# mkln/spamtree

Measured on AMD Instinct MI355X. Metric: Gibbs iterations/sec + achieved HBM GB/s, n=1e6 grid, 1/2/4/8 MI355X, higher is better.
Workload: dtype f64

## Files before the change

spamtree_amd/csrc/misc_kernels.hpp:

```cpp
#pragma once
#include "st_device.hpp"

struct LoglikArgs {
  const Blk *blks;
  const int *anc_idx;
  const int *list;
  int nlist;
  const double *panels;
  const double *w;
  double *loglik_c;
  double *resid;
  int maxP, maxM;
};

struct LoglikGrpArgs {
  const Blk *blks;
  const int *anc_idx;
  const Grp *grps;
  const int *list;
  int nlist;
  const double *panels;
  const double *w;
  double *loglik_c;
  int maxP;
// ... 176 lines not shown
  for (int i = lo + threadIdx.x; i < hi; i += NT) { xa += a[i]; xb += b[i]; }
  sa[threadIdx.x] = xa; sb[threadIdx.x] = xb;
  __syncthreads();
  for (int s2 = NT / 2; s2 > 0; s2 >>= 1) {
    if ((int)threadIdx.x < s2) { sa[threadIdx.x] += sa[threadIdx.x + s2]; sb[threadIdx.x] += sb[threadIdx.x + s2]; }
    __syncthreads();
  }
  if (threadIdx.x == 0) { partial[2 * blockIdx.x] = sa[0]; partial[2 * blockIdx.x + 1] = sb[0]; }
}
__global__ void k_sum2_final(const double *partial, double *out) {
  if (threadIdx.x < 2) {
    double s2 = 0.0;
    for (int g = 0; g < SUM2_WG; ++g) s2 += partial[2 * g + threadIdx.x];
    out[threadIdx.x] = s2;
  }
}

__global__ void k_xb(const double *X, const int *mv, const double *B, long long n, int p, double *xb) {
  const long long i = (long long)blockIdx.x * blockDim.x + threadIdx.x;
  if (i >= n) return;
  const double *bj = B + (size_t)p * mv[i];
  double acc = 0.0;
  for (int j = 0; j < p; ++j) acc += X[(size_t)j * n + i] * bj[j];
  xb[i] = acc;
}

template <int Q, bool XTX>
__global__ __launch_bounds__(NT) void k_stats(const double *X, const double *y, const double *w, const double *xb, const int *mv,
                                               const unsigned char *obs, const long long *partner, const double *wt, long long n,
                                               int p, double *partial) {
// ... 153 lines not shown
  const long long i = (long long)blockIdx.x * blockDim.x + threadIdx.x;
  if (i < n) buf[i] = mask[i] ? w[i] : 0.0;
  if (i < world) buf[n + i] = (i == rank && err[0] != INT_MAX) ? (double)err[0] : 0.0;
}

__global__ void k_merge_err(int *err, const int *err2) {
  if (threadIdx.x == 0 && blockIdx.x == 0 && err2[0] < err[0]) err[0] = err2[0];
}

#else
__global__ void k_normals(double *z, const long long *dev2model, long long n, unsigned iter, unsigned stream, unsigned long long seed);
__global__ void k_loglik(LoglikArgs A);
__global__ void k_loglik_grp(LoglikGrpArgs A);
__global__ void k_sum2_partial(const double *a, const double *b, int n, double *partial);
__global__ void k_sum2_final(const double *partial, double *out);
__global__ void k_xb(const double *X, const int *mv, const double *B, long long n, int p, double *xb);
template <int Q, bool XTX> __global__ void k_stats(const double *X, const double *y, const double *w, const double *xb, const int *mv, const unsigned char *obs, const long long *partner, const double *wt, long long n, int p, double *partial);
__global__ void k_stats_final(const double *partial, int nwg, int nq, double *out);
__global__ void k_yhat(const double *xb, const double *w, const double *noise, const int *mv, long long n, const double *tsq_inv_q, double *yhat);
__global__ void k_cross_cov(const double *c1, const int *mv1, long long n1, const double *c2, const int *mv2, long long n2, CovPar cp, double *out);
__global__ void k_qtile(QtArgs A);
__global__ void k_axpy_sum(double *acc, const double *x, long long n);
__global__ void k_pack_comps(const double *logdet, const double *loglik, const unsigned char *mask, int nb, const int *err, int rank, int world, double *buf);
__global__ void k_gather_pack(const double *w, const int *idx, int cnt, const int *err, double *out);
__global__ void k_gather_unpack(const double *recv, const int *idx, int cnt, long long total, double *w, double *errs);
__global__ void k_pack_w(const double *w, const unsigned char *mask, long long n, const int *err, int rank, int world, double *buf);
__global__ void k_merge_err(int *err, const int *err2);
#endif

static void launch_sum2(hipStream_t st, const double *a, const double *b, int n, double *partial, double *out) {
  hipLaunchKernelGGL(k_sum2_partial, dim3(SUM2_WG), dim3(NT), 0, st, a, b, n, partial);
  hipLaunchKernelGGL(k_sum2_final, dim3(1), dim3(64), 0, st, partial, out);
}
```

spamtree_amd/csrc/spamtree_hip.hip:

```cpp

#include "st_handle.hpp"
#include "misc_kernels.hpp"
#include "draw_store.hpp"
#include "rows_score.hpp"
#include <new>

static thread_local std::string g_create_error;
void points_free(st_handle_s *h);

enum RouteCode : int {
  R_NONE = ST_ROUTE_NONE,
  R_MARGINAL_INVCHOL_WAVE, R_MARGINAL_INVCHOL,
  R_FACTOR_LDS, R_FACTOR_SCRATCH, R_PREDICT_LDS, R_PREDICT_SCRATCH,
  R_QUAD32_REF_WCH, R_QUAD32_REF, R_QUAD32_LEAF, R_QUAD38_REF_WCH, R_QUAD38_REF, R_QUAD38_LEAF,
  R_QUAD44_REF_WCH, R_QUAD44_REF, R_QUAD44_LEAF, R_QUAD50_REF_WCH, R_QUAD50_REF, R_QUAD50_LEAF,
  R_FACTOR_MFMA, R_LCHAIN96, R_LCHAIN136, R_REF_FINISH, R_LCHAIN_SCALARS, R_FACTOR_WIDE, R_BIGMFMA3, R_BIGMFMA4, R_BIGMFMA5,
  R_GRAM, R_GRAM_DIRECT, R_GRAM_BIG,
  R_SAMPLE_MFMA, R_LEAF_SEG4, R_LEAF_SEG6, R_SAMPLE_LEAF, R_SAMPLE_WAVE, R_SAMPLE_LEAN_LAT, R_SAMPLE_LEAN,
  R_SAMPLE_BIG_REF, R_SAMPLE_LEAF_WIDE, R_SAMPLE_BIG_LEAF, R_SAMPLE_SMALL,
  R_COUNT
};
static const char *const k_route_names[R_COUNT] = {
  "",
  "k_marginal_invchol_wave", "k_marginal_invchol",
// ... 42 lines not shown
  return tab[size][kind];
}
static int launch_quad(int nkx, bool isref, bool wave_chol, int nquad, size_t lds, hipStream_t st, const QuadArgs &F, const CovPar &cp) {
  const int size = nkx == 32 ? 0 : nkx == 38 ? 1 : nkx == 44 ? 2 : 3, kind = isref ? (wave_chol ? 0 : 1) : 2;
  hipLaunchKernelGGL(quad_kernel(size, kind), dim3(nquad), dim3(128 * 4), lds, st, F, cp);
  return R_QUAD32_REF_WCH + QUAD_KINDS * size + kind;
}

static void invalidate_stats(st_handle_s *h) {
  if (h->stats_on_stream2) {
    (void)hipSetDevice(h->device);
    (void)hipStreamWaitEvent(h->stream, h->ev_stats, 0);
    h->stats_on_stream2 = false;
  }
  h->stats_valid = false; h->host_stats_valid = false;
}


extern "C" const char *st_last_error(st_handle h) { return h ? h->err.c_str() : g_create_error.c_str(); }
extern "C" void st_set_create_error(const char *msg) { g_create_error = msg ? msg : ""; }

extern "C" int st_destroy(st_handle h) {
  if (!h) return ST_OK;
  (void)hipSetDevice(h->device);
  if (h->ev_top) (void)hipEventDestroy(h->ev_top);
  if (h->ev_main) (void)hipEventDestroy(h->ev_main);
  if (h->ev_stats) (void)hipEventDestroy(h->ev_stats);
  if (h->stream2) (void)hipStreamDestroy(h->stream2);
  prof_harvest(h);
  for (auto e : h->ev_free) (void)hipEventDestroy(e);
  if (h->comm) (void)ncclCommDestroy(h->comm);
  if (h->pin) (void)hipHostFree(h->pin);
  if (h->pin_up) (void)hipHostFree(h->pin_up);
  for (int i = 0; i < 2; ++i) if (h->ev_up[i]) (void)hipEventDestroy(h->ev_up[i]);
  if (h->ev_factor) (void)hipEventDestroy(h->ev_factor);
  points_free(h);
  if (h->stream && !h->ext_stream) (void)hipStreamDestroy(h->stream);
  delete h;
  return ST_OK;
}

extern "C" int st_shard_plan_opt(const st_problem *pb, const st_options *opt_in, int32_t world, int64_t *owner, int32_t *cut_level) {
// ... 53 lines not shown
  for (long long r = 0; r < n; ++r)
    if (std::isfinite(pb->y[r])) rank_av[r] = t++;
  for (long long i = 0; i < n; ++i) {
    const long long r = h->dev2model[i];
    partner[i] = (h->quirks && rank_av[r] >= 0) ? h->model2dev[rank_av[r]] : i;
  }
  h->xtx.assign((size_t)pb->p * pb->p * pb->q, 0.0);
  for (long long r = 0; pb->p <= 8 && r < n; ++r) {
    if (!std::isfinite(pb->y[r])) continue;
    const int v = (int)(pb->mv_id[r] - 1);
    for (int a = 0; a < pb->p; ++a)
      for (int b2 = 0; b2 < pb->p; ++b2)
        h->xtx[(size_t)v * pb->p * pb->p + (size_t)b2 * pb->p + a] += pb->X[(size_t)a * n + r] * pb->X[(size_t)b2 * n + r];
  }
  CCHK(hipStreamCreate(&h->stream));
  CCHK(hipHostMalloc((void **)&h->pin, sizeof(PinnedArea), hipHostMallocDefault));
  new (h->pin) PinnedArea();
  h->pin_up_len = QMAX + std::max(1, h->p * h->q);
  CCHK(hipHostMalloc((void **)&h->pin_up, (size_t)2 * h->pin_up_len * sizeof(double), hipHostMallocDefault));
  for (int i = 0; i < 2; ++i) CCHK(hipEventCreateWithFlags(&h->ev_up[i], hipEventDisableTiming));
  CCHK(hipEventCreateWithFlags(&h->ev_factor, hipEventDisableTiming));
  CCHK(h->d_cx.upload(cx)); CCHK(h->d_cy.upload(cy)); CCHK(h->d_y.upload(y)); CCHK(h->d_X.upload(X));
  CCHK(h->d_mv.upload(mv)); CCHK(h->d_obs.upload(obs)); CCHK(h->d_partner.upload(partner));
  CCHK(h->d_dev2model.upload(h->dev2model));
  return ST_OK;
}

static int create_layout_buffers(st_handle_s *h) {
  {
    std::vector<Blk> db = h->blks;
    if (h->limited) for (Blk &B : db) B.acc_len = 0;
    CCHK(h->d_blks.upload(db));
// ... 33 lines not shown
  CCHK(h->d_resid.alloc(n));
  CCHK(hipMemset(h->d_resid.p, 0, n * sizeof(double)));
  CCHK(h->d_B.alloc((size_t)h->p * h->q));
  CCHK(h->d_tsq.alloc(QMAX));
  for (int s = 0; s < 2; ++s) {
    CCHK(h->d_panels[s].alloc(h->panel_total + 128));
    CCHK(hipMemset(h->d_panels[s].p, 0, (h->panel_total + 128) * sizeof(double)));
    CCHK(h->d_logdet[s].alloc(nb)); CCHK(h->d_loglik[s].alloc(nb));
    CCHK(hipMemset(h->d_logdet[s].p, 0, nb * sizeof(double)));
    CCHK(hipMemset(h->d_loglik[s].p, 0, nb * sizeof(double)));
  }
  CCHK(h->d_acc.alloc(std::max<size_t>(h->acc_total, 1)));
  CCHK(hipMemset(h->d_acc.p, 0, std::max<size_t>(h->acc_total, 1) * sizeof(double)));
  CCHK(h->d_scalars.alloc(8 + 2 * SUM2_WG));
  CCHK(h->d_err.alloc(2));
  CCHK(h->d_partial.alloc((size_t)STATS_WG * (h->p * h->q + h->q)));
  CCHK(h->d_stats.alloc((size_t)h->p * h->q + h->q));
  if (h->p <= 8) return ST_OK;
  const int p = h->p, pq = p * h->q;
  CCHK(h->d_xtx.alloc((size_t)p * pq));
  for (int b2 = 0; b2 < p; ++b2) {
    launch_stats(h, h->stream, h->d_X.p + (size_t)b2 * n);
    hipLaunchKernelGGL(k_stats_final, dim3(pq), dim3(NT), 0, h->stream, h->d_partial.p, STATS_WG, pq + h->q, h->d_xtx.p + (size_t)b2 * pq);
  }
  CCHK(hipGetLastError());
  std::vector<double> t((size_t)p * pq);
  CCHK(hipMemcpyAsync(t.data(), h->d_xtx.p, t.size() * sizeof(double), hipMemcpyDeviceToHost, h->stream));
  CCHK(hipStreamSynchronize(h->stream));
  h->d_xtx.free();
  for (int v = 0; v < h->q; ++v)
// ... 10 lines not shown
                        (const void *)k_sample<true, true>, (const void *)k_loglik, (const void *)k_factor_mfma, (const void *)k_factor_wide<WG_JT>,
                        (const void *)k_factor_ref_finish, (const void *)k_factor_bigmfma<5, 3, 24>, (const void *)k_factor_bigmfma<3, 5, 34>,
                        (const void *)k_factor_bigmfma<4, 5, 34>, (const void *)k_sample_mfma, (const void *)k_sample_wave,
                        (const void *)k_marginal_invchol, (const void *)k_marginal_invchol_wave})
    dyn(f, lim);
  dyn((const void *)k_factor_lchain<96>, (int)(lc_dyn_doubles(96) * 8));
  dyn((const void *)k_factor_lchain<136>, (int)(lc_dyn_doubles(136) * 8));
  for (int size = QUAD_SIZES - 1; size >= 0; --size)
    for (int kind = 0; kind < QUAD_KINDS; ++kind) dyn((const void *)quad_kernel(size, kind), cu - (int)dl.quad_static);
  h->async_top = h->g_top > 0 && h->sw.async_top;
  if (h->async_top) {
    CCHK(hipStreamCreateWithFlags(&h->stream2, hipStreamNonBlocking));
    CCHK(hipEventCreateWithFlags(&h->ev_top, hipEventDisableTiming));
    CCHK(hipEventCreateWithFlags(&h->ev_main, hipEventDisableTiming));
    CCHK(hipEventCreateWithFlags(&h->ev_stats, hipEventDisableTiming));
  }
  (void)hipGetLastError();
  return ST_OK;
}
#undef CCHK

extern "C" int st_create(const st_problem *pb, const st_options *opt, st_handle *out) {
  if (!pb || !out) { g_create_error = "st_create: null argument"; return ST_ERR_USAGE; }
  *out = nullptr;
  st_handle_s *h = new st_handle_s();
  h->device = opt ? opt->device : 0;
  h->quirks = opt ? opt->reference_quirks : 1;
  h->cache_gram = !(opt && (opt->reserved & 1));
  for (int j = 0; j < QMAX; ++j) h->tausq_inv[j] = 1.0;
  std::string msg;
// ... 83 lines not shown
  HCHK(h, hipGetLastError());
  return ST_OK;
}
extern "C" int st_set_tausq_inv(st_handle h, const double *t) {
  if (!h || !t) return ST_ERR_USAGE;
  for (int j = 0; j < h->q; ++j) h->tausq_inv[j] = t[j];
  HCHK(h, hipSetDevice(h->device));
  h->pin_up_slot ^= 1;
  HCHK(h, hipEventSynchronize(h->ev_up[h->pin_up_slot]));
  double *stg = h->pin_up + (size_t)h->pin_up_slot * h->pin_up_len;
  std::memcpy(stg, h->tausq_inv, QMAX * sizeof(double));
  HCHK(h, hipMemcpyAsync(h->d_tsq.p, stg, QMAX * sizeof(double), hipMemcpyHostToDevice, h->stream));
  HCHK(h, hipEventRecord(h->ev_up[h->pin_up_slot], h->stream));
  return ST_OK;
}
static int settle_top(st_handle h) {
  if (h->top_pending) { HCHK(h, hipSetDevice(h->device)); HCHK(h, hipStreamWaitEvent(h->stream, h->ev_top, 0)); }
  return ST_OK;
}
static QuadArgs quad_args(st_handle h, int grp_first, long long qr_off, int qr_words, int nquad, int ldS, int phys, int *errflag) {
  QuadArgs F;
  std::memset(&F, 0, sizeof(F));
  F.blks = h->d_blks.p; F.anc_idx = h->d_anc.p; F.grps = h->d_grps.p + grp_first;
  F.qrec = qr_off >= 0 ? h->d_qrec.p + qr_off : nullptr; F.qrec_stride = qr_words; F.nquad = nquad;
  F.cx = h->d_cx.p; F.cy = h->d_cy.p; F.mv = h->d_mv.p; F.w = h->d_w.p; F.panels = h->d_panels[phys].p;
  F.errflag = errflag; F.ldS = ldS;
  F.g_in = h->d_resid.p;
  return F;
}
static int complete_leaf(st_handle h, int slot) {
  const int phys = h->slot_map[slot];
  if (!h->leaf_pending[phys]) return ST_OK;
  HCHK(h, hipSetDevice(h->device));
  const CovPar &cp = h->leaf_cp[phys];
  ProfScope phase(h, 0, -2, 0);
  for (int g = 0; g < h->n_actual_groups; ++g) {
    const LevelInfo &L = h->levels[g];
    if (L.vl_off < 0) continue;
    QuadArgs F = quad_args(h, L.grp_first, L.qr_off, L.qr_words, L.qown_n, L.q_ldS, phys, h->d_err.p);
    F.wave_chol = L.maxM <= 27 ? 1 : 0;
    F.mode = QM_TFROMV; F.vscr = h->d_vleaf.p + L.vl_off; F.vtiles = quad_vtiles(L.q_nkx);
    ProfScope ps(h, 0, g, 0);
    (void)launch_quad(L.q_nkx, false, true, L.qown_n, L.lds_quad, h->stream, F, cp);
    HCHK(h, hipGetLastError());
  }
  h->leaf_pending[phys] = false;
  return ST_OK;
}
extern "C" int st_swap(st_handle h) {
  if (!h) return ST_ERR_USAGE;
  if (const int rc = refuse_factor_open(h, "st_swap")) return rc;
  if (const int rc = refuse_sweep_pending(h, "st_swap")) return rc;
  if (h->top_pending) {
    h->err = "st_swap between st_factor_begin and the st_factor / st_factor_local that picks its result up";
// ... 61 lines not shown

static bool uses_exchange(st_handle h) { return h->world > 1 || h->comm; }
static int refuse_without_comm(st_handle h, const char *alternatives) {
  h->err = std::string("world > 1: call st_comm_init first, or use ") + alternatives;
  return ST_ERR_USAGE;
}
static int enqueue_result(st_handle h, const double *a, const double *b, int n, Landing *dst) {
  {
    ProfScope ps(h, 3);
    launch_sum2(h->stream, a, b, n, h->d_scalars.p + 8, h->d_scalars.p);
  }
  HCHK(h, hipGetLastError());
  HCHK(h, hipMemcpyAsync(dst->sums, h->d_scalars.p, 2 * sizeof(double), hipMemcpyDeviceToHost, h->stream));
  return ST_OK;
}
static int enqueue_slot_result(st_handle h, int slot, Landing *dst) {
  const int phys = h->slot_map[slot];
  return enqueue_result(h, h->d_logdet[phys].p, h->d_loglik[phys].p, (int)h->n_blocks, dst);
}
static int enqueue_comm_result(st_handle h, Landing *dst, double *rank_words) {
  const int nb = (int)h->n_blocks;
  if (const int rc = enqueue_result(h, h->d_comm.p, h->d_comm.p + nb, nb, dst)) return rc;
  HCHK(h, hipMemcpyAsync(rank_words, h->d_comm.p + 2 * (size_t)nb, h->world * sizeof(double), hipMemcpyDeviceToHost, h->stream));
  return ST_OK;
}
static int enqueue_fail_word(st_handle h, Landing *dst) {
  HCHK(h, hipMemcpyAsync(dst->err, h->d_err.p, 2 * sizeof(int), hipMemcpyDeviceToHost, h->stream));
  return ST_OK;
}
static int reset_err(st_handle h) {
  const int init[2] = {INT_MAX, 0};
  HCHK(h, hipMemcpyAsync(h->d_err.p, init, 2 * sizeof(int), hipMemcpyHostToDevice, h->stream));
  return ST_OK;
}


static int factor_launch(st_handle h, int phys, const CovPar &cp, int g_lo = 0, int g_hi = INT_MAX, hipStream_t st = nullptr, int *errflag = nullptr,
                         bool vonly = false, bool *deferred = nullptr) {
  g_hi = std::min(g_hi, h->n_actual_groups);
  if (!st) st = h->stream;
  if (!errflag) errflag = h->d_err.p;
  int n_launch = 0;
  for (int g = g_lo; g < g_hi; ++g) n_launch += ((h->levels[g].fast ? h->levels[g].gown_n : h->levels[g].own_n) != 0);
  ProfScope phase(h, 0, -2, n_launch, st);
  for (int g = g_lo; g < g_hi; ++g) std::fill_n(h->route_a.begin() + (size_t)g * ST_ROUTE_A_SLOTS, ST_ROUTE_A_SLOTS, (int)R_NONE);
  auto route = [&](int g, int code) {
    int *r = h->route_a.data() + (size_t)g * ST_ROUTE_A_SLOTS;
    for (int i = 0; i < ST_ROUTE_A_SLOTS; ++i) if (r[i] == R_NONE) { r[i] = code; return; }
  };
  if (g_lo == 0 && h->limited && !h->twin_list.empty()) {
    MarginalArgs M;
    M.blks = h->d_blks.p; M.list = h->d_twin.p; M.nlist = (int)h->twin_list.size(); M.cx = h->d_cx.p; M.cy = h->d_cy.p; M.mv = h->d_mv.p;
    M.panels = h->d_panels[phys].p; M.errflag = errflag; M.maxM = h->twin_maxM;
    M.w = h->d_w.p; M.resid = h->d_resid.p;
    const size_t lds = (size_t)2 * h->twin_maxM * h->twin_maxM * sizeof(double);
    if (h->twin_maxM <= 27 && !h->force_generic) {
// ... 90 lines not shown
  CovPar cp;
  int rc = make_covpar(h, theta, ntheta, &cp);
  if (rc) return rc;
  if (h->top_pending) HCHK(h, hipStreamWaitEvent(h->stream2, h->ev_top, 0));
  HCHK(h, hipEventRecord(h->ev_main, h->stream));
  HCHK(h, hipStreamWaitEvent(h->stream2, h->ev_main, 0));
  const int init[2] = {INT_MAX, 0};
  HCHK(h, hipMemcpyAsync(h->d_err2.p, init, 2 * sizeof(int), hipMemcpyHostToDevice, h->stream2));
  const int phys = h->slot_map[slot];
  h->leaf_pending[phys] = false;
  h->prof_suspend = true;
  rc = factor_launch(h, phys, cp, 0, h->g_top, h->stream2, h->d_err2.p);
  h->prof_suspend = false;
  if (rc) return rc;
  HCHK(h, hipEventRecord(h->ev_top, h->stream2));
  h->top_pending = true; h->top_phys = phys; h->top_theta.assign(theta, theta + ntheta);
  return ST_OK;
}
static int fix_top_comps(st_handle h, int phys);
static int run_stats(st_handle h, hipStream_t st);
static int stats_begin(st_handle h) {
  if (!h->stream2 || h->stats_valid) return ST_OK;
  HCHK(h, hipEventRecord(h->ev_main, h->stream));
  HCHK(h, hipStreamWaitEvent(h->stream2, h->ev_main, 0));
  int rc = run_stats(h, h->stream2);
  if (rc) return rc;
  const size_t nq = (size_t)h->p * h->q + h->q;
  h->stats_prefetched = nq <= (size_t)ST_PIN_STATS;
  if (h->stats_prefetched) HCHK(h, hipMemcpyAsync(h->pin->stats, h->d_stats.p, nq * sizeof(double), hipMemcpyDeviceToHost, h->stream2));
  HCHK(h, hipEventRecord(h->ev_stats, h->stream2));
  h->stats_on_stream2 = true;
  return ST_OK;
}

// ... 9 lines not shown
  int rc = make_covpar(h, theta, ntheta, &cp);
  if (rc) return rc;
  h->theta[slot].assign(theta, theta + ntheta);
  if (slot == 0) { h->gram_valid = false; std::fill(h->s0_valid.begin(), h->s0_valid.end(), 0); }
  rc = reset_err(h);
  if (rc) return rc;
  const int phys = h->slot_map[slot];
  h->leaf_pending[phys] = false;
  if (slot == 1) { rc = stats_begin(h); if (rc) return rc; }
  bool reuse = false;
  if (h->top_pending) {
    HCHK(h, hipStreamWaitEvent(h->stream, h->ev_top, 0));
    reuse = h->top_phys == phys && (int)h->top_theta.size() == ntheta && std::equal(theta, theta + ntheta, h->top_theta.begin());
    h->top_pending = false;
  }
  if (reuse) { rc = fix_top_comps(h, phys); if (rc) return rc; }
  bool deferred = false;
  rc = factor_launch(h, phys, cp, reuse ? h->g_top : 0, INT_MAX, nullptr, nullptr, vonly, &deferred);
  if (deferred) { h->leaf_pending[phys] = true; h->leaf_cp[phys] = cp; }
  if (rc || !reuse) return rc;
  hipLaunchKernelGGL(k_merge_err, dim3(1), dim3(64), 0, h->stream, h->d_err.p, h->d_err2.p);
  HCHK(h, hipGetLastError());
  return ST_OK;
}

extern "C" int st_mg_pack_comps(st_handle h, int slot, void **dev_ptr, int64_t *len) {
  if (!h || slot < 0 || slot > 1) return ST_ERR_USAGE;
  HCHK(h, hipSetDevice(h->device));
  { const int rc0 = settle_top(h); if (rc0) return rc0; }
  const int phys = h->slot_map[slot], nb = (int)h->n_blocks;
  {
    ProfScope ps(h, 3);
    hipLaunchKernelGGL(k_pack_comps, dim3((std::max(nb, h->world) + NT - 1) / NT), dim3(NT), 0, h->stream, h->d_logdet[phys].p,
                       h->d_loglik[phys].p, h->d_blkmask.p, nb, h->d_err.p, h->rank, h->world, h->d_comm.p);
  }
  HCHK(h, hipGetLastError());
// ... 62 lines not shown
  return st_factor_finish(h, loglik);
}
extern "C" int st_factor_is_async(st_handle h) { return (h && !uses_exchange(h)) ? 1 : 0; }
extern "C" int st_factor_enqueue(st_handle h, int slot, const double *theta, int ntheta) {
  return factor_enqueue(h, slot, theta, ntheta, h && h->defer_leaf && slot == 1);
}
static int factor_enqueue(st_handle h, int slot, const double *theta, int ntheta, bool vonly) {
  if (!h || !theta || slot < 0 || slot > 1) return ST_ERR_USAGE;
  if (h->factor_open) { h->err = "st_factor_enqueue: the previous one has not been finished"; return ST_ERR_USAGE; }
  if (uses_exchange(h)) {
    h->factor_open = true; h->factor_open_slot = slot; h->top_theta_open.assign(theta, theta + ntheta);
    return ST_OK;
  }
  int rc = factor_local(h, slot, theta, ntheta, vonly);
  if (rc) return rc;
  if ((rc = enqueue_slot_result(h, slot, &h->pin->factor)) || (rc = enqueue_fail_word(h, &h->pin->factor))) return rc;
  HCHK(h, hipEventRecord(h->ev_factor, h->stream));
  h->factor_open = true; h->factor_open_slot = slot; h->top_theta_open.clear();
  return ST_OK;
}
extern "C" int st_factor_finish(st_handle h, double *loglik) {
  if (!h) return ST_ERR_USAGE;
  if (!h->factor_open) { h->err = "st_factor_finish without st_factor_enqueue"; return ST_ERR_USAGE; }
  h->factor_open = false;
  if (uses_exchange(h)) {
    if (!h->comm) return refuse_without_comm(h, "st_factor_local / st_mg_pack_comps / (all-reduce) / st_mg_finish");
    int rc = st_factor_local(h, h->factor_open_slot, h->top_theta_open.data(), (int)h->top_theta_open.size());
    if (rc) return rc;
    return exchange_comps_and_finish(h, h->factor_open_slot, loglik);
  }
  HCHK(h, hipSetDevice(h->device));
  HCHK(h, hipEventSynchronize(h->ev_factor));
  return landing_code(h->pin->factor, loglik);
}

static int enqueue_sweep_loglik(st_handle h, const double *z, uint64_t seed, uint32_t iter, int slot, Landing *dst) {
  int rc = st_sample_w_local(h, z, seed, iter);
  if (rc) return rc;
  rc = st_sample_w_top(h);
  if (rc) return rc;
  rc = enqueue_fail_word(h, dst);
  if (rc) return rc;
  rc = st_loglik_local(h, slot);
  if (rc) return rc;
  return enqueue_slot_result(h, slot, dst);
}

static int gather_w_scatter(st_handle h);
static int sweep_exchange(st_handle h, const double *z, uint64_t seed, uint32_t iter, void **send, void **recv, int64_t *count) {
  int rc = st_sample_w_local(h, z, seed, iter);
  if (rc) return rc;
  if (h->top_len > 0) {
    ProfScope ps(h, 7);
    NCHK(h, ncclAllReduce(h->d_acc.p + h->top_off, h->d_acc.p + h->top_off, (size_t)h->top_len, ncclDouble, ncclSum, h->comm, h->stream));
  }
  rc = st_sample_w_top(h);
  if (rc) return rc;
  return st_mg_gather_w_pack(h, send, recv, count);
}

// ... 83 lines not shown
  HCHK(h, hipGetLastError());
  return ST_OK;
}

static int sample_launch(st_handle h, int g_hi, int g_lo) {
  const int phys = h->slot_map[0];
  for (int g = g_hi - 1; g >= g_lo; --g) {
    const LevelInfo &L = h->levels[g];
    int *route = h->route_b.data() + 2 * (size_t)g;
    route[0] = route[1] = R_NONE;
    if ((L.fast ? L.gown_n : L.own_n) == 0) continue;
    SampleArgs A;
    std::memset(&A, 0, sizeof(A));
    A.blks = h->d_blks.p; A.anc_idx = h->d_anc.p; A.dch_idx = h->d_dch.p; A.list = h->d_lvl.p + L.first + L.own_lo; A.nlist = L.own_n;
    A.panels = h->d_panels[phys].p; A.w = h->d_w.p; A.y = h->d_y.p; A.xb = h->d_xb.p; A.z = h->d_z.p; A.mv = h->d_mv.p;
    A.obs = h->d_obs.p; A.acc = h->d_acc.p; A.errflag = h->d_err.p; A.maxP = L.maxP; A.maxM = L.maxM; A.maxLd = L.maxLd;
    for (int j = 0; j < QMAX; ++j) A.tausq_inv[j] = h->tausq_inv[j];
    A.do_gram = (h->gram_valid && h->cache_gram) ? 0 : 1;
    A.no_fwd = h->limited ? 1 : 0;
    A.lds_sq = (L.big_sample && L.sample_sq) ? 2 : 0;
    A.s0 = h->d_s0.p; A.s0off = h->d_s0off.p;
    {
      ProfScope ps(h, 1, h->n_actual_groups + g);
      if (L.fast) {
        SampleFastArgs F;
        std::memset(&F, 0, sizeof(F));
        F.do_gram = A.do_gram; F.no_fwd = A.no_fwd;
        F.blks = h->d_blks.p; F.anc_idx = h->d_anc.p; F.dch_idx = h->d_dch.p; F.grps = h->d_grps.p + L.grp_first + L.gown_lo; F.ngrp = L.gown_n;
        F.panels = h->d_panels[phys].p; F.w = h->d_w.p; F.y = h->d_y.p; F.xb = h->d_xb.p; F.z = h->d_z.p; F.mv = h->d_mv.p;
        F.acc = h->d_acc.p; F.errflag = h->d_err.p; F.ldN = L.ldN; F.Mr4 = L.Mr4; F.Mrows = L.Mrows; F.maxP = L.maxP; F.av_dbl = L.av_dbl;
        F.gdesc = h->d_gdesc.p + (size_t)(L.grp_first + L.gown_lo) * h->gd_stride; F.gd_stride = h->gd_stride;
        for (int j = 0; j < QMAX; ++j) F.tausq_inv[j] = h->tausq_inv[j];
        const bool lean_ok = h->sw.sample_lean && !(!L.isref && L.maxP > 255);
        F.gdesc_all = h->d_gdesc.p;
        auto splits = [&](int gq) {
          const LevelInfo &Lq = h->levels[gq];
          const bool lean_q = h->sw.sample_lean && !(!Lq.isref && Lq.maxP > 255);
          return Lq.fast && lean_q && h->sw.split_gram && (h->sw.split_gram == 2 || (Lq.isref && Lq.gown_n >= 32 * h->sm_count));
        };
        const bool direct_parent = F.do_gram && h->gram_direct_level == g && splits(g) && h->levels[g + 1].gown_n > 0;
        if (F.do_gram && lean_ok && g == h->gram_direct_level + 1 && h->gram_direct_level >= 0 && splits(g - 1) && h->levels[g - 1].gown_n > 0) F.do_gram = 0;
        if (F.do_gram && lean_ok && h->sw.split_gram && (h->sw.split_gram == 2 || (L.isref && L.gown_n >= 32 * h->sm_count))) {
          if (direct_parent) { route[0] = R_GRAM_DIRECT; hipLaunchKernelGGL(k_gram_direct, dim3(L.gown_n), dim3(NT), 0, h->stream, F); }
          else { route[0] = R_GRAM; hipLaunchKernelGGL(k_gram, dim3(L.gown_n), dim3(NT), 0, h->stream, F); }
          F.do_gram = 0;
// ... 150 lines not shown
    return st_mg_gather_w_unpack(h);
  }
  int rc = st_sample_w_local(h, z, seed, iter);
  if (rc) return rc;
  rc = st_sample_w_top(h);
  if (rc) return rc;
  Landing res;
  rc = enqueue_fail_word(h, &res);
  if (rc) return rc;
  HCHK(h, hipStreamSynchronize(h->stream));
  return landing_code(res, nullptr);
}

extern "C" int st_loglik_local(st_handle h, int slot) {
  if (!h || slot < 0 || slot > 1) return ST_ERR_USAGE;
  HCHK(h, hipSetDevice(h->device));
  if (slot == 1) { const int rc0 = settle_top(h); if (rc0) return rc0; }
  { const int rc0 = complete_leaf(h, slot); if (rc0) return rc0; }
  const int phys = h->slot_map[slot];
  int maxP = 0, maxM = 0;
  for (auto &L : h->levels) { maxP = std::max(maxP, L.maxP); maxM = std::max(maxM, L.maxM); }
  const size_t lds = lds_loglik_bytes(maxP, maxM);
  LoglikArgs A;
  A.blks = h->d_blks.p; A.anc_idx = h->d_anc.p; A.list = h->d_ownslow.p; A.nlist = (int)h->own_obs_slow.size();
  A.panels = h->d_panels[phys].p; A.w = h->d_w.p; A.loglik_c = h->d_loglik[phys].p; A.resid = nullptr; A.maxP = maxP; A.maxM = maxM;
  {
    ProfScope ps(h, 2);
    if (A.nlist > 0) hipLaunchKernelGGL(k_loglik, dim3(A.nlist), dim3(NT), lds, h->stream, A);
    if (!h->own_grp_list.empty()) {
      LoglikGrpArgs Gr;
      Gr.blks = h->d_blks.p; Gr.anc_idx = h->d_anc.p; Gr.grps = h->d_grps.p; Gr.list = h->d_owngrp.p; Gr.nlist = (int)h->own_grp_list.size();
      Gr.panels = h->d_panels[phys].p; Gr.w = h->d_w.p; Gr.loglik_c = h->d_loglik[phys].p; Gr.maxP = maxP;
      Gr.gdesc = h->d_gdesc.p; Gr.gd_stride = h->gd_stride;
      hipLaunchKernelGGL(k_loglik_grp, dim3(Gr.nlist), dim3(NT), (size_t)(maxP + 32) * sizeof(double), h->stream, Gr);
    }
  }
  HCHK(h, hipGetLastError());
  HCHK(h, reset_err(h) == ST_OK ? hipSuccess : hipErrorUnknown);
  return ST_OK;
}
static int fix_top_comps(st_handle h, int phys) {
  if (h->n_toplist == 0) return ST_OK;
  int maxP = 0, maxM = 0;
  for (int g = 0; g < h->g_top; ++g) { maxP = std::max(maxP, h->levels[g].maxP); maxM = std::max(maxM, h->levels[g].maxM); }
  LoglikArgs A;
  A.blks = h->d_blks.p; A.anc_idx = h->d_anc.p; A.list = h->d_toplist.p; A.nlist = h->n_toplist;
  A.panels = h->d_panels[phys].p; A.w = h->d_w.p; A.loglik_c = h->d_loglik[phys].p; A.resid = h->d_resid.p; A.maxP = maxP; A.maxM = maxM;
  {
    ProfScope ps(h, 0, h->g_top > 0 ? h->g_top - 1 : 0);
    hipLaunchKernelGGL(k_loglik, dim3(A.nlist), dim3(NT), lds_loglik_bytes(maxP, maxM), h->stream, A);
  }
  HCHK(h, hipGetLastError());
  return ST_OK;
}
extern "C" int st_loglik_w(st_handle h, int slot, double *loglik) {
  if (!h) return ST_ERR_USAGE;
  if (slot >= 0 && slot <= 1) { if (const int rc = refuse_factor_open(h, "st_loglik_w", slot)) return rc; }
  if (const int rc = refuse_sweep_pending(h, "st_loglik_w")) return rc;
  if (slot >= 0 && slot <= 1) { const int rc0 = complete_leaf(h, slot); if (rc0) return rc0; }
  if (uses_exchange(h)) {
    if (!h->comm) return refuse_without_comm(h, "st_loglik_local / st_mg_pack_comps / (all-reduce) / st_mg_finish");
    int rc = st_loglik_local(h, slot);
    if (rc) return rc;
    return exchange_comps_and_finish(h, slot, loglik);
  }
  int rc = st_loglik_local(h, slot);
  if (rc) return rc;
  Landing res;
  rc = enqueue_slot_result(h, slot, &res);
  if (rc) return rc;
  HCHK(h, hipStreamSynchronize(h->stream));
  return landing_code(res, loglik);
}

extern "C" int st_predict(st_handle h, int theta_changed) {
  (void)theta_changed;
  if (!h) return ST_ERR_USAGE;
  if (const int rc = refuse_factor_open(h, "st_predict")) return rc;
  if (const int rc = refuse_sweep_pending(h, "st_predict")) return rc;
  if (h->pred_list.empty()) return ST_OK;
  invalidate_stats(h);
  if (!h->z_valid) { h->err = "st_predict needs the normals of a preceding st_sample_w (spamtree_model.cpp:1325)"; return ST_ERR_USAGE; }
  if (h->theta[0].empty()) { h->err = "st_predict before st_factor(slot 0)"; return ST_ERR_USAGE; }
  HCHK(h, hipSetDevice(h->device));
  CovPar cp;
  int rc = make_covpar(h, h->theta[0].data(), (int)h->theta[0].size(), &cp);
  if (rc) return rc;
  const LevelInfo &L = h->pred_info;
  if (h->pred_nkx > 0 && h->pred_quad_count > 0) {
    QuadArgs F = quad_args(h, h->pred_grp_first, h->pred_qr_off, h->pred_qr_words, h->pred_quad_count, quad_lds_stride(h->pred_nkx), h->slot_map[0], h->d_err.p);
    F.wave_chol = 1; F.predict = 1; F.z = h->d_z.p; F.w_out = h->d_w.p;
    {
      ProfScope ps(h, 6);
      h->route_p = launch_quad(h->pred_nkx, false, true, h->pred_quad_count, h->pred_lds, h->stream, F, cp);
    }
    HCHK(h, hipGetLastError());
    HCHK(h, hipStreamSynchronize(h->stream));
    return ST_OK;
  }
  FactorArgs A;
  std::memset(&A, 0, sizeof(A));
  A.blks = h->d_blks.p; A.anc_idx = h->d_anc.p; A.list = h->d_pred.p; A.nlist = (int)h->pred_list.size();
  A.cx = h->d_cx.p; A.cy = h->d_cy.p; A.mv = h->d_mv.p; A.w_in = h->d_w.p; A.w_out = h->d_w.p; A.z = h->d_z.p;
  A.panels = h->d_panels[h->slot_map[0]].p; A.logdet_c = nullptr; A.loglik_c = nullptr; A.errflag = h->d_err.p;
  A.maxP = L.maxP; A.maxM = L.maxM; A.maxMa = L.maxMa; A.SR = L.big_factor ? 4 : 8;
  {
    ProfScope ps(h, 6);
    if (L.big_factor) { h->route_p = R_PREDICT_SCRATCH; launch_factor<true, MODE_PREDICT>(h, L, A, cp); }
    else { h->route_p = R_PREDICT_LDS; launch_factor<false, MODE_PREDICT>(h, L, A, cp); }
  }
  HCHK(h, hipGetLastError());
  HCHK(h, hipStreamSynchronize(h->stream));
  return ST_OK;
}

static int run_stats(st_handle h, hipStream_t st = nullptr) {
  const int nq = h->p * h->q + h->q;
  if (h->stats_valid) return ST_OK;
  if (!st) st = h->stream;
// ... 924 lines not shown
```

spamtree_amd/csrc/st_handle.hpp:

```cpp
#pragma once
#include "tree_layout.hpp"
#include "st_protocol.hpp"
#include "simulate_kernels.hpp"
#include "loo_layout.hpp"
#include "loo_kernels.hpp"
#include "psis_kernels.hpp"

template <typename T>
struct DevBuf {
  T *p = nullptr;
  size_t n = 0;
  DevBuf() = default;
  DevBuf(const DevBuf &) = delete;
  DevBuf &operator=(const DevBuf &) = delete;
  DevBuf(DevBuf &&o) noexcept : p(o.p), n(o.n) { o.p = nullptr; o.n = 0; }
  DevBuf &operator=(DevBuf &&o) noexcept { if (this != &o) { free(); p = o.p; n = o.n; o.p = nullptr; o.n = 0; } return *this; }
  ~DevBuf() { free(); }
  hipError_t alloc(size_t count) {
    n = count;
    if (count == 0) { p = nullptr; return hipSuccess; }
    return hipMalloc((void **)&p, count * sizeof(T));
  }
  hipError_t upload(const std::vector<T> &v) {
    hipError_t e = alloc(v.size());
// ... 18 lines not shown
  DevBuf<double> d_lcrow;
  DevBuf<double> d_s0;
  DevBuf<long long> d_s0off;
  bool c_pending = false;
  int c_rc = 0; double c_ll = 0.0;
  DevBuf<int> d_ownobs, d_owngrp, d_ownslow;
  DevBuf<unsigned char> d_rowmask, d_blkmask;
  DevBuf<double> d_comm;
  DevBuf<double> d_gather;
  DevBuf<int> d_gidx;
  DevBuf<double> d_gerr;
  hipStream_t stream2 = nullptr;
  hipEvent_t ev_top = nullptr, ev_main = nullptr;
  DevBuf<int> d_err2, d_toplist;
  bool async_top = false, top_pending = false, prof_suspend = false, async_top_off = false;
  hipEvent_t ev_stats = nullptr;
  bool stats_on_stream2 = false;
  bool stats_prefetched = false;
  int top_phys = -1;
  std::vector<double> top_theta;
  bool ext_stream = false;
  DevBuf<double> d_sum_w, d_sum_yhat;
  long long n_summary = 0;
  DevBuf<double> d_draws_w, d_draws_yhat;
  long long draws_cap = 0, n_draws = 0;
  DevBuf<double> d_rs_tgt, d_rs_hold;
  DevBuf<double> d_rs_acc, d_rs_rows, d_rs_crps, d_rs_partial, d_rs_tot;
  bool rs_set = false;
  long long rs_n_acc = 0, rs_n_tgt = 0, rs_n_held = 0;
  std::vector<long long> rs_nobs_q, rs_nheld_q;
// ... 5 lines not shown
  DevBuf<long long> d_loo_voff;
  DevBuf<double> d_loo_S, d_loo_last, d_loo_acc, d_loo_rows, d_loo_tot;
  std::vector<LooLevelLaunch> loo_levels;
  double loo_bytes = 0, loo_flops = 0;
  bool loo_set = false;
  int loo_mask = 0;
  long long loo_n_acc = 0, loo_fin_acc = -1;
  std::vector<long long> loo_nobs_q;
  DevBuf<double> d_loo_store, d_psis_rows, d_psis_tot;
  DevBuf<int> d_psis_int;
  long long loo_keep = 0, psis_fin_acc = -1;
  bool stats_valid = false;
  bool host_stats_valid = false;
  std::vector<double> host_stats;
  PinnedArea *pin = nullptr;
  double *pin_up = nullptr;
  int pin_up_slot = 0, pin_up_len = 0;
  hipEvent_t ev_up[2] = {nullptr, nullptr};
  bool factor_open = false; int factor_open_slot = 0;
  std::vector<double> top_theta_open;
  hipEvent_t ev_factor = nullptr;
  std::vector<char> s0_valid;
  bool gram_valid = false;
  bool cache_gram = true;
  bool leaf_pending[2] = {false, false};
  CovPar leaf_cp[2];
  DevBuf<double> d_vleaf;
  DevBuf<double> d_resid;
  DevBuf<int> d_twin;
  ncclComm_t comm = nullptr;
// ... 84 lines not shown
```

spamtree_amd/csrc/st_protocol.hpp:

```cpp
#pragma once
#include <climits>
#include <cstddef>

constexpr int ST_MAX_RANKS = 64;
constexpr int ST_PIN_STATS = 40;

struct Landing {
  double sums[2] = {0.0, 0.0};
  int err[2] = {INT_MAX, 0};
};

struct PinnedArea {
  Landing sweep;
  Landing deferred;
  Landing factor;
  double stats[ST_PIN_STATS];
};

inline int landing_code(const Landing &L, double *loglik) {
  if (L.err[0] != INT_MAX) return L.err[0] & 15;
  if (loglik) *loglik = L.sums[0] + L.sums[1];
  return 0;
}

inline int rank_failure(const double *words, int world) {
  int best = INT_MAX;
  for (int r = 0; r < world; ++r)
    if (words[r] > 0.5 && (int)words[r] < best) best = (int)words[r];
  return best == INT_MAX ? 0 : (best & 15);
}
```

Before: 259.0.

## Fuse result landing into one kernel writing mapped pinned memory, overlap top loglik

Replaces the per-iteration sum2 partial/final kernels, device-to-host memcpys of sums and error word, and the host-to-device error reset with a single last-block-ticket reduction kernel. That kernel writes sums and error directly into mapped coherent host memory and resets the error word on device. It also moves the top-level k_loglik fix-up onto the second stream so it overlaps the main loglik, and skips redundant error resets using a small tracker. This cuts small copies and launches per Gibbs iteration, at the cost of atomics and ticket logic and a dependency on coherent mapped host memory.

```diff
diff --git a/profiles/micro/landing_gaps.py b/profiles/micro/landing_gaps.py
--- /dev/null
+++ b/profiles/micro/landing_gaps.py
@@ -0,0 +1,98 @@
+import csv
+import re
+import sys
+from collections import Counter
+
+
+def short(name):
+    name = re.sub(r"^void ", "", name)
+    m = re.match(r"([A-Za-z_0-9:() ]*?k_[a-z_0-9]+(<[^>]*>)?)", name)
+    return m.group(1) if m else name.split("(")[0][:40]
+
+
+BIG = ("k_factor", "k_sample", "k_gram", "k_loglik_grp", "k_marginal")
+
+
+def is_big(n):
+    return n.startswith(BIG)
+
+
+def main(path):
+    rows = []
+    with open(path, newline="") as f:
+        for r in csv.DictReader(f):
+            rows.append((int(r["Start_Timestamp"]), int(r["End_Timestamp"]), short(r["Kernel_Name"])))
+    rows.sort()
+    anchors = [i for i, r in enumerate(rows) if r[2] == "k_loglik_grp"]
+    if len(anchors) < 3:
+        sys.exit("no iterations found")
+
+    def uncovered(t0, t1):
+        segs = sorted((max(s, t0), min(e, t1)) for s, e, n in rows if is_big(n) and e > t0 and s < t1)
+        cov, cur = 0, t0
+        for s, e in segs:
+            if e > cur:
+                cov += e - max(s, cur)
+                cur = e
+        return (t1 - t0) - cov
+
+    def ops(t0, t1):
+        return [n for s, e, n in rows if t0 <= s < t1 and not is_big(n)]
+
+    acc = {k: [] for k in "abc"}
+    opc = {k: Counter() for k in "abc"}
+    copies = []
+    for ai, a in enumerate(anchors[1:-1], 1):
+        gs, ge, _ = rows[a]
+        j = a - 1
+        while j >= 0 and not rows[j][2].startswith("k_sample"):
+            j -= 1
+        ta = max(r[1] for r in rows[max(0, j - 8):j + 1] if r[2].startswith(("k_sample", "k_gram")))
+        j = a + 1
+        while j < len(rows) and not rows[j][2].startswith("k_factor_quad"):
+            j += 1
+        tb = rows[j][0]
+        nxt = anchors[ai + 1]
+        k = j
+        stop = next((i for i in range(j, nxt) if rows[i][2] == "k_normals"), nxt)
+        leaf = max((i for i in range(j, stop) if rows[i][2].startswith("k_factor_quad")), key=lambda i: rows[i][1])
+        quads = [i for i in range(j, stop) if rows[i][2].startswith("k_factor_quad")]
+        leaf = quads[min(3, len(quads) - 1)]
+        tl = rows[leaf][1]
+        tail = [i for i in range(leaf + 1, stop) if rows[i][0] >= tl]
+        tc = None
+        for p, i in enumerate(tail):
+            if rows[i][2].startswith("k_landing"):
+                tc = rows[i][1]
+                break
+            if rows[i][2] == "k_sum2_final":
+                cp = [x for x in tail[p + 1:] if "copyBuffer" in rows[x][2]][:2]
+                tc = rows[cp[-1]][1]
+                break
+        if tc is None:
+            continue
+        for key, t0, t1 in (("a", ta, gs), ("b", ge, tb), ("c", tl, tc)):
+            acc[key].append((t1 - t0, uncovered(t0, t1)))
+            opc[key].update(ops(t0, t1))
+        copies.append(sum(1 for s, e, n in rows[a:nxt] if "copyBuffer" in n))
+    n = len(copies)
+    print(f"{n} iterations")
+    for key in "abc":
+        ln = sum(x[0] for x in acc[key]) / n / 1e3
+        un = sum(x[1] for x in acc[key]) / n / 1e3
+        print(f"({key}) length {ln:7.1f} us, not covered by phase A/B/C kernels {un:7.1f} us; operations per iteration: "
+              + ", ".join(f"{v / n:.2f} {k}" for k, v in opc[key].most_common()))
+    print(f"small copies (blit kernels) per iteration: {sum(copies) / n:.2f}")
+    ov = 0
+    tot = 0
+    for a in anchors[1:-1]:
+        gs, ge, _ = rows[a]
+        for s, e, nme in rows[max(0, a - 6):a + 12]:
+            if nme == "k_loglik":
+                tot += 1
+                ov += (s < ge and e > gs)
+    print(f"k_loglik launches that overlap k_loglik_grp: {ov} of {tot}")
+
+
+if __name__ == "__main__":
+    main(sys.argv[1])
diff --git a/spamtree_amd/csrc/misc_kernels.hpp b/spamtree_amd/csrc/misc_kernels.hpp
--- a/spamtree_amd/csrc/misc_kernels.hpp
+++ b/spamtree_amd/csrc/misc_kernels.hpp
@@ -1,5 +1,6 @@
 #pragma once
 #include "st_device.hpp"
+#include "st_protocol.hpp"
 
 struct LoglikArgs {
   const Blk *blks;
@@ -214,6 +215,38 @@
     for (int g = 0; g < SUM2_WG; ++g) s2 += partial[2 * g + threadIdx.x];
     out[threadIdx.x] = s2;
   }
+}
+
+__global__ __launch_bounds__(NT) void k_landing(const double *a, const double *b, int n, double *partial, unsigned *ticket, int *err,
+                                                Landing *dst) {
+  __shared__ double sa[NT], sb[NT];
+  __shared__ int s_last;
+  const int chunk = (n + SUM2_WG - 1) / SUM2_WG;
+  const int lo = blockIdx.x * chunk, hi = min(n, lo + chunk);
+  double xa = 0.0, xb = 0.0;
+  for (int i = lo + threadIdx.x; i < hi; i += NT) { xa += a[i]; xb += b[i]; }
+  sa[threadIdx.x] = xa; sb[threadIdx.x] = xb;
+  __syncthreads();
+  for (int s2 = NT / 2; s2 > 0; s2 >>= 1) {
+    if ((int)threadIdx.x < s2) { sa[threadIdx.x] += sa[threadIdx.x + s2]; sb[threadIdx.x] += sb[threadIdx.x + s2]; }
+    __syncthreads();
+  }
+  if (threadIdx.x == 0) {
+    __hip_atomic_store(partial + 2 * blockIdx.x, sa[0], __ATOMIC_RELAXED, __HIP_MEMORY_SCOPE_AGENT);
+    __hip_atomic_store(partial + 2 * blockIdx.x + 1, sb[0], __ATOMIC_RELAXED, __HIP_MEMORY_SCOPE_AGENT);
+    __threadfence();
+    asm volatile("s_waitcnt vmcnt(0)" ::: "memory");
+    s_last = atomicAdd(ticket, 1u) == gridDim.x - 1;
+  }
+  __syncthreads();
+  if (!s_last || threadIdx.x >= 2) return;
+  __threadfence();
+  double s2 = 0.0;
+  for (int g = 0; g < SUM2_WG; ++g) s2 += __hip_atomic_load(partial + 2 * g + threadIdx.x, __ATOMIC_RELAXED, __HIP_MEMORY_SCOPE_AGENT);
+  dst->sums[threadIdx.x] = s2;
+  dst->err[threadIdx.x] = __hip_atomic_load(err + threadIdx.x, __ATOMIC_RELAXED, __HIP_MEMORY_SCOPE_AGENT);
+  err[threadIdx.x] = threadIdx.x == 0 ? INT_MAX : 0;
+  if (threadIdx.x == 0) __hip_atomic_store(ticket, 0u, __ATOMIC_RELAXED, __HIP_MEMORY_SCOPE_AGENT);
 }
 
 __global__ void k_xb(const double *X, const int *mv, const double *B, long long n, int p, double *xb) {
@@ -397,6 +430,7 @@
 __global__ void k_loglik_grp(LoglikGrpArgs A);
 __global__ void k_sum2_partial(const double *a, const double *b, int n, double *partial);
 __global__ void k_sum2_final(const double *partial, double *out);
+__global__ void k_landing(const double *a, const double *b, int n, double *partial, unsigned *ticket, int *err, Landing *dst);
 __global__ void k_xb(const double *X, const int *mv, const double *B, long long n, int p, double *xb);
 template <int Q, bool XTX> __global__ void k_stats(const double *X, const double *y, const double *w, const double *xb, const int *mv, const unsigned char *obs, const long long *partner, const double *wt, long long n, int p, double *partial);
 __global__ void k_stats_final(const double *partial, int nwg, int nq, double *out);
@@ -415,3 +449,6 @@
   hipLaunchKernelGGL(k_sum2_partial, dim3(SUM2_WG), dim3(NT), 0, st, a, b, n, partial);
   hipLaunchKernelGGL(k_sum2_final, dim3(1), dim3(64), 0, st, partial, out);
 }
+static void launch_landing(hipStream_t st, const double *a, const double *b, int n, double *partial, unsigned *ticket, int *err, Landing *dst) {
+  hipLaunchKernelGGL(k_landing, dim3(SUM2_WG), dim3(NT), 0, st, a, b, n, partial, ticket, err, dst);
+}
diff --git a/spamtree_amd/csrc/spamtree_hip.hip b/spamtree_amd/csrc/spamtree_hip.hip
--- a/spamtree_amd/csrc/spamtree_hip.hip
+++ b/spamtree_amd/csrc/spamtree_hip.hip
@@ -80,6 +80,7 @@
     h->stats_on_stream2 = false;
   }
   h->stats_valid = false; h->host_stats_valid = false;
+  h->top_fixed = false;
 }
 
 
@@ -92,6 +93,7 @@
   if (h->ev_top) (void)hipEventDestroy(h->ev_top);
   if (h->ev_main) (void)hipEventDestroy(h->ev_main);
   if (h->ev_stats) (void)hipEventDestroy(h->ev_stats);
+  if (h->ev_w) (void)hipEventDestroy(h->ev_w);
   if (h->stream2) (void)hipStreamDestroy(h->stream2);
   prof_harvest(h);
   for (auto e : h->ev_free) (void)hipEventDestroy(e);
@@ -175,8 +177,9 @@
         h->xtx[(size_t)v * pb->p * pb->p + (size_t)b2 * pb->p + a] += pb->X[(size_t)a * n + r] * pb->X[(size_t)b2 * n + r];
   }
   CCHK(hipStreamCreate(&h->stream));
-  CCHK(hipHostMalloc((void **)&h->pin, sizeof(PinnedArea), hipHostMallocDefault));
+  CCHK(hipHostMalloc((void **)&h->pin, sizeof(PinnedArea), hipHostMallocMapped | hipHostMallocCoherent));
   new (h->pin) PinnedArea();
+  CCHK(hipHostGetDevicePointer((void **)&h->pin_dev, h->pin, 0));
   h->pin_up_len = QMAX + std::max(1, h->p * h->q);
   CCHK(hipHostMalloc((void **)&h->pin_up, (size_t)2 * h->pin_up_len * sizeof(double), hipHostMallocDefault));
   for (int i = 0; i < 2; ++i) CCHK(hipEventCreateWithFlags(&h->ev_up[i], hipEventDisableTiming));
@@ -240,6 +243,8 @@
   CCHK(hipMemset(h->d_acc.p, 0, std::max<size_t>(h->acc_total, 1) * sizeof(double)));
   CCHK(h->d_scalars.alloc(8 + 2 * SUM2_WG));
   CCHK(h->d_err.alloc(2));
+  CCHK(h->d_ticket.alloc(1));
+  CCHK(hipMemset(h->d_ticket.p, 0, sizeof(unsigned)));
   CCHK(h->d_partial.alloc((size_t)STATS_WG * (h->p * h->q + h->q)));
   CCHK(h->d_stats.alloc((size_t)h->p * h->q + h->q));
   if (h->p <= 8) return ST_OK;
@@ -280,6 +285,7 @@
     CCHK(hipEventCreateWithFlags(&h->ev_top, hipEventDisableTiming));
     CCHK(hipEventCreateWithFlags(&h->ev_main, hipEventDisableTiming));
     CCHK(hipEventCreateWithFlags(&h->ev_stats, hipEventDisableTiming));
+    CCHK(hipEventCreateWithFlags(&h->ev_w, hipEventDisableTiming));
   }
   (void)hipGetLastError();
   return ST_OK;
@@ -393,6 +399,7 @@
   HCHK(h, hipEventRecord(h->ev_up[h->pin_up_slot], h->stream));
   return ST_OK;
 }
+static int *err_word(st_handle h) { h->errw.wrote(); return h->d_err.p; }
 static int settle_top(st_handle h) {
   if (h->top_pending) { HCHK(h, hipSetDevice(h->device)); HCHK(h, hipStreamWaitEvent(h->stream, h->ev_top, 0)); }
   return ST_OK;
@@ -416,7 +423,7 @@
   for (int g = 0; g < h->n_actual_groups; ++g) {
     const LevelInfo &L = h->levels[g];
     if (L.vl_off < 0) continue;
-    QuadArgs F = quad_args(h, L.grp_first, L.qr_off, L.qr_words, L.qown_n, L.q_ldS, phys, h->d_err.p);
+    QuadArgs F = quad_args(h, L.grp_first, L.qr_off, L.qr_words, L.qown_n, L.q_ldS, phys, err_word(h));
     F.wave_chol = L.maxM <= 27 ? 1 : 0;
     F.mode = QM_TFROMV; F.vscr = h->d_vleaf.p + L.vl_off; F.vtiles = quad_vtiles(L.q_nkx);
     ProfScope ps(h, 0, g, 0);
@@ -508,23 +515,32 @@
   HCHK(h, hipMemcpyAsync(dst->sums, h->d_scalars.p, 2 * sizeof(double), hipMemcpyDeviceToHost, h->stream));
   return ST_OK;
 }
-static int enqueue_slot_result(st_handle h, int slot, Landing *dst) {
-  const int phys = h->slot_map[slot];
-  return enqueue_result(h, h->d_logdet[phys].p, h->d_loglik[phys].p, (int)h->n_blocks, dst);
-}
 static int enqueue_comm_result(st_handle h, Landing *dst, double *rank_words) {
   const int nb = (int)h->n_blocks;
   if (const int rc = enqueue_result(h, h->d_comm.p, h->d_comm.p + nb, nb, dst)) return rc;
   HCHK(h, hipMemcpyAsync(rank_words, h->d_comm.p + 2 * (size_t)nb, h->world * sizeof(double), hipMemcpyDeviceToHost, h->stream));
   return ST_OK;
 }
+static int enqueue_landing(st_handle h, int slot, Landing *dst) {
+  const int phys = h->slot_map[slot];
+  Landing *dev = (Landing *)((char *)h->pin_dev + ((char *)dst - (char *)h->pin));
+  {
+    ProfScope ps(h, 3);
+    launch_landing(h->stream, h->d_logdet[phys].p, h->d_loglik[phys].p, (int)h->n_blocks, h->d_scalars.p + 8, h->d_ticket.p, h->d_err.p, dev);
+  }
+  HCHK(h, hipGetLastError());
+  h->errw.landed();
+  return ST_OK;
+}
 static int enqueue_fail_word(st_handle h, Landing *dst) {
   HCHK(h, hipMemcpyAsync(dst->err, h->d_err.p, 2 * sizeof(int), hipMemcpyDeviceToHost, h->stream));
   return ST_OK;
 }
 static int reset_err(st_handle h) {
+  if (!h->errw.needs_reset()) return ST_OK;
   const int init[2] = {INT_MAX, 0};
   HCHK(h, hipMemcpyAsync(h->d_err.p, init, 2 * sizeof(int), hipMemcpyHostToDevice, h->stream));
+  h->errw.reset_done();
   return ST_OK;
 }
 
@@ -533,7 +549,7 @@
                          bool vonly = false, bool *deferred = nullptr) {
   g_hi = std::min(g_hi, h->n_actual_groups);
   if (!st) st = h->stream;
-  if (!errflag) errflag = h->d_err.p;
+  if (!errflag) errflag = err_word(h);
   int n_launch = 0;
   for (int g = g_lo; g < g_hi; ++g) n_launch += ((h->levels[g].fast ? h->levels[g].gown_n : h->levels[g].own_n) != 0);
   ProfScope phase(h, 0, -2, n_launch, st);
@@ -654,10 +670,12 @@
   h->prof_suspend = false;
   if (rc) return rc;
   HCHK(h, hipEventRecord(h->ev_top, h->stream2));
-  h->top_pending = true; h->top_phys = phys; h->top_theta.assign(theta, theta + ntheta);
-  return ST_OK;
-}
-static int fix_top_comps(st_handle h, int phys);
+  h->top_pending = true; h->top_fixed = false; h->top_phys = phys; h->top_theta.assign(theta, theta + ntheta);
+  return ST_OK;
+}
+static int fix_top_comps(st_handle h, int phys, hipStream_t st = nullptr);
+static int fix_top_ahead(st_handle h);
+static int loglik_launch(st_handle h, int slot);
 static int run_stats(st_handle h, hipStream_t st);
 static int stats_begin(st_handle h) {
   if (!h->stream2 || h->stats_valid) return ST_OK;
@@ -697,12 +715,13 @@
     reuse = h->top_phys == phys && (int)h->top_theta.size() == ntheta && std::equal(theta, theta + ntheta, h->top_theta.begin());
     h->top_pending = false;
   }
-  if (reuse) { rc = fix_top_comps(h, phys); if (rc) return rc; }
+  if (reuse && !h->top_fixed) { rc = fix_top_comps(h, phys); if (rc) return rc; }
+  h->top_fixed = false;
   bool deferred = false;
   rc = factor_launch(h, phys, cp, reuse ? h->g_top : 0, INT_MAX, nullptr, nullptr, vonly, &deferred);
   if (deferred) { h->leaf_pending[phys] = true; h->leaf_cp[phys] = cp; }
   if (rc || !reuse) return rc;
-  hipLaunchKernelGGL(k_merge_err, dim3(1), dim3(64), 0, h->stream, h->d_err.p, h->d_err2.p);
+  hipLaunchKernelGGL(k_merge_err, dim3(1), dim3(64), 0, h->stream, err_word(h), h->d_err2.p);
   HCHK(h, hipGetLastError());
   return ST_OK;
 }
@@ -795,7 +814,7 @@
   }
   int rc = factor_local(h, slot, theta, ntheta, vonly);
   if (rc) return rc;
-  if ((rc = enqueue_slot_result(h, slot, &h->pin->factor)) || (rc = enqueue_fail_word(h, &h->pin->factor))) return rc;
+  if ((rc = enqueue_landing(h, slot, &h->pin->factor))) return rc;
   HCHK(h, hipEventRecord(h->ev_factor, h->stream));
   h->factor_open = true; h->factor_open_slot = slot; h->top_theta_open.clear();
   return ST_OK;
@@ -820,11 +839,11 @@
   if (rc) return rc;
   rc = st_sample_w_top(h);
   if (rc) return rc;
-  rc = enqueue_fail_word(h, dst);
-  if (rc) return rc;
-  rc = st_loglik_local(h, slot);
-  if (rc) return rc;
-  return enqueue_slot_result(h, slot, dst);
+  rc = fix_top_ahead(h);
+  if (rc) return rc;
+  rc = loglik_launch(h, slot);
+  if (rc) return rc;
+  return enqueue_landing(h, slot, dst);
 }
 
 static int gather_w_scatter(st_handle h);
@@ -938,7 +957,7 @@
     std::memset(&A, 0, sizeof(A));
     A.blks = h->d_blks.p; A.anc_idx = h->d_anc.p; A.dch_idx = h->d_dch.p; A.list = h->d_lvl.p + L.first + L.own_lo; A.nlist = L.own_n;
     A.panels = h->d_panels[phys].p; A.w = h->d_w.p; A.y = h->d_y.p; A.xb = h->d_xb.p; A.z = h->d_z.p; A.mv = h->d_mv.p;
-    A.obs = h->d_obs.p; A.acc = h->d_acc.p; A.errflag = h->d_err.p; A.maxP = L.maxP; A.maxM = L.maxM; A.maxLd = L.maxLd;
+    A.obs = h->d_obs.p; A.acc = h->d_acc.p; A.errflag = err_word(h); A.maxP = L.maxP; A.maxM = L.maxM; A.maxLd = L.maxLd;
     for (int j = 0; j < QMAX; ++j) A.tausq_inv[j] = h->tausq_inv[j];
     A.do_gram = (h->gram_valid && h->cache_gram) ? 0 : 1;
     A.no_fwd = h->limited ? 1 : 0;
@@ -952,7 +971,7 @@
         F.do_gram = A.do_gram; F.no_fwd = A.no_fwd;
         F.blks = h->d_blks.p; F.anc_idx = h->d_anc.p; F.dch_idx = h->d_dch.p; F.grps = h->d_grps.p + L.grp_first + L.gown_lo; F.ngrp = L.gown_n;
         F.panels = h->d_panels[phys].p; F.w = h->d_w.p; F.y = h->d_y.p; F.xb = h->d_xb.p; F.z = h->d_z.p; F.mv = h->d_mv.p;
-        F.acc = h->d_acc.p; F.errflag = h->d_err.p; F.ldN = L.ldN; F.Mr4 = L.Mr4; F.Mrows = L.Mrows; F.maxP = L.maxP; F.av_dbl = L.av_dbl;
+        F.acc = h->d_acc.p; F.errflag = A.errflag; F.ldN = L.ldN; F.Mr4 = L.Mr4; F.Mrows = L.Mrows; F.maxP = L.maxP; F.av_dbl = L.av_dbl;
         F.gdesc = h->d_gdesc.p + (size_t)(L.grp_first + L.gown_lo) * h->gd_stride; F.gd_stride = h->gd_stride;
         for (int j = 0; j < QMAX; ++j) F.tausq_inv[j] = h->tausq_inv[j];
         const bool lean_ok = h->sw.sample_lean && !(!L.isref && L.maxP > 255);
@@ -1133,6 +1152,10 @@
 
 extern "C" int st_loglik_local(st_handle h, int slot) {
   if (!h || slot < 0 || slot > 1) return ST_ERR_USAGE;
+  if (const int rc = loglik_launch(h, slot)) return rc;
+  return reset_err(h);
+}
+static int loglik_launch(st_handle h, int slot) {
   HCHK(h, hipSetDevice(h->device));
   if (slot == 1) { const int rc0 = settle_top(h); if (rc0) return rc0; }
   { const int rc0 = complete_leaf(h, slot); if (rc0) return rc0; }
@@ -1155,21 +1178,31 @@
     }
   }
   HCHK(h, hipGetLastError());
-  HCHK(h, reset_err(h) == ST_OK ? hipSuccess : hipErrorUnknown);
-  return ST_OK;
-}
-static int fix_top_comps(st_handle h, int phys) {
+  return ST_OK;
+}
+static int fix_top_comps(st_handle h, int phys, hipStream_t st) {
   if (h->n_toplist == 0) return ST_OK;
+  if (!st) st = h->stream;
   int maxP = 0, maxM = 0;
   for (int g = 0; g < h->g_top; ++g) { maxP = std::max(maxP, h->levels[g].maxP); maxM = std::max(maxM, h->levels[g].maxM); }
   LoglikArgs A;
   A.blks = h->d_blks.p; A.anc_idx = h->d_anc.p; A.list = h->d_toplist.p; A.nlist = h->n_toplist;
   A.panels = h->d_panels[phys].p; A.w = h->d_w.p; A.loglik_c = h->d_loglik[phys].p; A.resid = h->d_resid.p; A.maxP = maxP; A.maxM = maxM;
   {
-    ProfScope ps(h, 0, h->g_top > 0 ? h->g_top - 1 : 0);
-    hipLaunchKernelGGL(k_loglik, dim3(A.nlist), dim3(NT), lds_loglik_bytes(maxP, maxM), h->stream, A);
+    ProfScope ps(h, 0, h->g_top > 0 ? h->g_top - 1 : 0, 1, st);
+    hipLaunchKernelGGL(k_loglik, dim3(A.nlist), dim3(NT), lds_loglik_bytes(maxP, maxM), st, A);
   }
   HCHK(h, hipGetLastError());
+  return ST_OK;
+}
+static int fix_top_ahead(st_handle h) {
+  if (!h->stream2 || !h->top_pending || h->n_toplist == 0) return ST_OK;
+  HCHK(h, hipEventRecord(h->ev_w, h->stream));
+  HCHK(h, hipStreamWaitEvent(h->stream2, h->ev_w, 0));
+  const int rc = fix_top_comps(h, h->top_phys, h->stream2);
+  if (rc) return rc;
+  HCHK(h, hipEventRecord(h->ev_top, h->stream2));
+  h->top_fixed = true;
   return ST_OK;
 }
 extern "C" int st_loglik_w(st_handle h, int slot, double *loglik) {
@@ -1185,11 +1218,10 @@
   }
   int rc = st_loglik_local(h, slot);
   if (rc) return rc;
-  Landing res;
-  rc = enqueue_slot_result(h, slot, &res);
-  if (rc) return rc;
-  HCHK(h, hipStreamSynchronize(h->stream));
-  return landing_code(res, loglik);
+  rc = enqueue_landing(h, slot, &h->pin->sweep);
+  if (rc) return rc;
+  HCHK(h, hipStreamSynchronize(h->stream));
+  return landing_code(h->pin->sweep, loglik);
 }
 
 extern "C" int st_predict(st_handle h, int theta_changed) {
@@ -1207,7 +1239,7 @@
   if (rc) return rc;
   const LevelInfo &L = h->pred_info;
   if (h->pred_nkx > 0 && h->pred_quad_count > 0) {
-    QuadArgs F = quad_args(h, h->pred_grp_first, h->pred_qr_off, h->pred_qr_words, h->pred_quad_count, quad_lds_stride(h->pred_nkx), h->slot_map[0], h->d_err.p);
+    QuadArgs F = quad_args(h, h->pred_grp_first, h->pred_qr_off, h->pred_qr_words, h->pred_quad_count, quad_lds_stride(h->pred_nkx), h->slot_map[0], err_word(h));
     F.wave_chol = 1; F.predict = 1; F.z = h->d_z.p; F.w_out = h->d_w.p;
     {
       ProfScope ps(h, 6);
@@ -1221,7 +1253,7 @@
   std::memset(&A, 0, sizeof(A));
   A.blks = h->d_blks.p; A.anc_idx = h->d_anc.p; A.list = h->d_pred.p; A.nlist = (int)h->pred_list.size();
   A.cx = h->d_cx.p; A.cy = h->d_cy.p; A.mv = h->d_mv.p; A.w_in = h->d_w.p; A.w_out = h->d_w.p; A.z = h->d_z.p;
-  A.panels = h->d_panels[h->slot_map[0]].p; A.logdet_c = nullptr; A.loglik_c = nullptr; A.errflag = h->d_err.p;
+  A.panels = h->d_panels[h->slot_map[0]].p; A.logdet_c = nullptr; A.loglik_c = nullptr; A.errflag = err_word(h);
   A.maxP = L.maxP; A.maxM = L.maxM; A.maxMa = L.maxMa; A.SR = L.big_factor ? 4 : 8;
   {
     ProfScope ps(h, 6);
diff --git a/spamtree_amd/csrc/st_handle.hpp b/spamtree_amd/csrc/st_handle.hpp
--- a/spamtree_amd/csrc/st_handle.hpp
+++ b/spamtree_amd/csrc/st_handle.hpp
@@ -56,6 +56,8 @@
   hipEvent_t ev_top = nullptr, ev_main = nullptr;
   DevBuf<int> d_err2, d_toplist;
   bool async_top = false, top_pending = false, prof_suspend = false, async_top_off = false;
+  hipEvent_t ev_w = nullptr;
+  bool top_fixed = false;
   hipEvent_t ev_stats = nullptr;
   bool stats_on_stream2 = false;
   bool stats_prefetched = false;
@@ -91,6 +93,9 @@
   bool host_stats_valid = false;
   std::vector<double> host_stats;
   PinnedArea *pin = nullptr;
+  PinnedArea *pin_dev = nullptr;
+  DevBuf<unsigned> d_ticket;
+  ErrWordTracker errw;
   double *pin_up = nullptr;
   int pin_up_slot = 0, pin_up_len = 0;
   hipEvent_t ev_up[2] = {nullptr, nullptr};
diff --git a/spamtree_amd/csrc/st_protocol.hpp b/spamtree_amd/csrc/st_protocol.hpp
--- a/spamtree_amd/csrc/st_protocol.hpp
+++ b/spamtree_amd/csrc/st_protocol.hpp
@@ -17,6 +17,18 @@
   double stats[ST_PIN_STATS];
 };
 
+struct ErrWordTracker {
+  bool clean = false;
+  long long resets = 0, skipped = 0;
+  void wrote() { clean = false; }
+  void landed() { clean = true; }
+  bool needs_reset() {
+    if (clean) { ++skipped; return false; }
+    return true;
+  }
+  void reset_done() { clean = true; ++resets; }
+};
+
 inline int landing_code(const Landing &L, double *loglik) {
   if (L.err[0] != INT_MAX) return L.err[0] & 15;
   if (loglik) *loglik = L.sums[0] + L.sums[1];
```

Result: no change. 261.2, median of 6 (+0.9%).
